# darcamo/pyphysim

Measured on AMD Instinct MI355X. Metric: Monte Carlo realizations/sec (whole node) + SER abs-error vs ref, higher is better.
Workload: dtype f64

## Files before the change

### pyphysim_amd/csrc/capi.hip

```cpp
#include <cmath>
#include <cstdarg>

#include "common.hpp"
#include "modem.hpp"

namespace mcle {

static thread_local char g_err[512] = "";

void set_error(const char* fmt, ...) {
    va_list ap;
    va_start(ap, fmt);
    vsnprintf(g_err, sizeof(g_err), fmt, ap);
    va_end(ap);
}

}

using namespace mcle;

int mcle_ctx::bind() const {
    MCLE_HIP(hipSetDevice(device));
    return MCLE_OK;
}

int mcle_ctx::scratch(size_t bytes, void** d_ptr) {
    if (bytes > scratch_bytes) {
        if (d_scratch) MCLE_HIP(hipFree(d_scratch));
        d_scratch = nullptr;
        scratch_bytes = 0;
        size_t want = bytes < (1u << 20) ? (1u << 20) : (bytes < ((size_t)256 << 20) ? bytes + bytes / 4 : bytes);
        hipError_t e = hipMalloc(&d_scratch, want);
        if (e == hipErrorOutOfMemory && want > bytes) {
            (void)hipGetLastError();
            want = bytes;
            e = hipMalloc(&d_scratch, want);
        }
        if (e != hipSuccess) {
            d_scratch = nullptr;
            MCLE_HIP(e);
        }
        scratch_bytes = want;
    }
    *d_ptr = d_scratch;
    return MCLE_OK;
}

int mcle_ctx::scratch_upto(size_t want, size_t floor_bytes, void** d_ptr, size_t* got) {
    if (want <= scratch_bytes) {
        *d_ptr = d_scratch;
        *got = want;
        return MCLE_OK;
    }
    size_t free_b = 0, total_b = 0;
    if (hipMemGetInfo(&free_b, &total_b) == hipSuccess) {
        const size_t avail = free_b + scratch_bytes;
        const size_t margin = (size_t)256 << 20;
        if (avail > margin && want > avail - margin) want = avail - margin;
    } else {
        (void)hipGetLastError();
    }
    if (want < floor_bytes) want = floor_bytes;
    for (;;) {
        const int rc = scratch(want, d_ptr);
        if (rc == MCLE_OK) {
            *got = want;
            return MCLE_OK;
        }
        if (want <= floor_bytes) return rc;
        (void)hipGetLastError();
        want = want / 2 < floor_bytes ? floor_bytes : want / 2;
    }
}

int mcle_ctx::get_twiddles(int n, int dtype, void** d_tw) {
    TwiddleKey key{n, dtype};
    auto it = twiddles.find(key);
    if (it != twiddles.end()) {
        *d_tw = it->second;
        return MCLE_OK;
    }
    const double two_pi = 6.283185307179586476925286766559;
    void* d = nullptr;
    if (dtype == MCLE_F64) {
        std::vector<double2> h(n);
        for (int k = 0; k < n; ++k) {
            h[k].x = std::cos(two_pi * k / n);
            h[k].y = -std::sin(two_pi * k / n);
        }
        MCLE_HIP(hipMalloc(&d, n * sizeof(double2)));
        MCLE_HIP(hipMemcpy(d, h.data(), n * sizeof(double2), hipMemcpyHostToDevice));
    } else {
        std::vector<float2> h(n);
        for (int k = 0; k < n; ++k) {
            h[k].x = (float)std::cos(two_pi * k / n);
            h[k].y = (float)-std::sin(two_pi * k / n);
        }
        MCLE_HIP(hipMalloc(&d, n * sizeof(float2)));
        MCLE_HIP(hipMemcpy(d, h.data(), n * sizeof(float2), hipMemcpyHostToDevice));
    }
    twiddles[key] = d;
    *d_tw = d;
    return MCLE_OK;
}

extern "C" {

const char* mcle_last_error(void) { return g_err; }

int mcle_version(void) { return MCLE_VERSION; }

int mcle_device_count(int* count) {
    MCLE_REQUIRE(count != nullptr, "null output pointer");
    int n = 0;
    hipError_t e = hipGetDeviceCount(&n);
    if (e != hipSuccess) {
        (void)hipGetLastError();
        n = 0;
    }
    *count = n;
    return MCLE_OK;
}

int mcle_ctx_create(int device_id, mcle_ctx** out) {
    MCLE_REQUIRE(out != nullptr, "null output pointer");
    *out = nullptr;
    int n = 0;
    hipError_t e = hipGetDeviceCount(&n);
    if (e != hipSuccess || n <= 0) {
        (void)hipGetLastError();
        set_error("no HIP device available (hipGetDeviceCount: %s); libmcle has no CPU fallback",
                  e == hipSuccess ? "0 devices" : hipGetErrorString(e));
        return MCLE_E_HIP;
    }
    MCLE_REQUIRE(device_id >= 0 && device_id < n, "device_id %d out of range [0, %d)", device_id, n);
    MCLE_HIP(hipSetDevice(device_id));
    hipDeviceProp_t prop;
    MCLE_HIP(hipGetDeviceProperties(&prop, device_id));
    if (std::strncmp(prop.gcnArchName, "gfx950", 6) != 0) {
        set_error("device %d is %s; libmcle is built for gfx950 (MI355X) only", device_id, prop.gcnArchName);
        return MCLE_E_HIP;
    }
    mcle_ctx* ctx = new (std::nothrow) mcle_ctx();
    if (!ctx) {
        set_error("out of host memory");
        return MCLE_E_NOMEM;
    }
    ctx->device = device_id;
    ctx->n_cu = prop.multiProcessorCount;
    ctx->lds_bytes = (int)prop.sharedMemPerBlock;
    ctx->name = prop.name;
    hipError_t es = hipStreamCreateWithFlags(&ctx->stream, hipStreamNonBlocking);
    if (es != hipSuccess) {
        set_error("hipStreamCreate failed: %s", hipGetErrorString(es));
        delete ctx;
        return MCLE_E_HIP;
    }
    ctx->own_stream = true;
    (void)hipEventCreate(&ctx->ev0);
    (void)hipEventCreate(&ctx->ev1);
    (void)hipEventCreate(&ctx->ev_probe0);
    (void)hipEventCreate(&ctx->ev_probe1);
    *out = ctx;
    return MCLE_OK;
}

int mcle_ctx_destroy(mcle_ctx* ctx) {
    if (!ctx) return MCLE_OK;
    (void)hipSetDevice(ctx->device);
    (void)hipStreamSynchronize(ctx->stream);
    (void)mcle_comm_destroy(ctx);
    if (ctx->d_comm_buf) (void)hipFree(ctx->d_comm_buf);
    for (auto& kv : ctx->twiddles) (void)hipFree(kv.second);
    if (ctx->d_table_f32) (void)hipFree(ctx->d_table_f32);
    if (ctx->d_table_f64) (void)hipFree(ctx->d_table_f64);
    if (ctx->d_grid) (void)hipFree(ctx->d_grid);
    if (ctx->d_psk) (void)hipFree(ctx->d_psk);
    if (ctx->d_scratch) (void)hipFree(ctx->d_scratch);
    if (ctx->ev0) (void)hipEventDestroy(ctx->ev0);
    if (ctx->ev1) (void)hipEventDestroy(ctx->ev1);
    if (ctx->ev_probe0) (void)hipEventDestroy(ctx->ev_probe0);
    if (ctx->ev_probe1) (void)hipEventDestroy(ctx->ev_probe1);
    if (ctx->own_stream && ctx->stream) (void)hipStreamDestroy(ctx->stream);
    delete ctx;
    return MCLE_OK;
}

int mcle_ctx_set_stream(mcle_ctx* ctx, void* hip_stream) {
    MCLE_REQUIRE(ctx != nullptr, "null context");
    MCLE_HIP(hipSetDevice(ctx->device));
    MCLE_HIP(hipStreamSynchronize(ctx->stream));
    if (ctx->own_stream && ctx->stream) MCLE_HIP(hipStreamDestroy(ctx->stream));
    if (hip_stream) {
        ctx->stream = (hipStream_t)hip_stream;
        ctx->own_stream = false;
    } else {
        MCLE_HIP(hipStreamCreateWithFlags(&ctx->stream, hipStreamNonBlocking));
        ctx->own_stream = true;
    }
    return MCLE_OK;
}

int mcle_ctx_get_stream(mcle_ctx* ctx, void** hip_stream) {
    MCLE_REQUIRE(ctx != nullptr && hip_stream != nullptr, "null argument");
    *hip_stream = (void*)ctx->stream;
    return MCLE_OK;
}

int mcle_ctx_set_option(mcle_ctx* ctx, int option, long long value) {
    MCLE_REQUIRE(ctx != nullptr, "null context");
    MCLE_REQUIRE(option >= 0 && option < MCLE_OPT_COUNT, "unknown option %d", option);
    bool ok = false;
    switch (option) {
        case MCLE_OPT_NO_MFMA: case MCLE_OPT_SINGLE_TDL: case MCLE_OPT_JAKES_DIRECT: case MCLE_OPT_F64_GENERIC: case MCLE_OPT_BD_RUNTIME_SOLVE: case MCLE_OPT_DEMOD_NOCERT: case MCLE_OPT_F32_MFMA: case MCLE_OPT_WALK_LEGACY: case MCLE_OPT_STAGED_GENERIC: ok = value == 0 || value == 1; break;
        case MCLE_OPT_TDL_KERNEL: ok = value >= 0 && value <= 4; break;
#ifdef MCLE_EXPERIMENTS
        case MCLE_OPT_MIMO_TDL_KERNEL: ok = value >= 0 && value <= 255; break;
#else
        case MCLE_OPT_MIMO_TDL_KERNEL: ok = value >= 0 && value <= 2; break;
#endif
#ifdef MCLE_EXPERIMENTS
        case MCLE_OPT_F64_VARIANT: ok = value >= 0 && value <= 2047; break;
#else
        case MCLE_OPT_F64_VARIANT:
            MCLE_REQUIRE(value == 0, "option MCLE_OPT_F64_VARIANT: the timing-bound variants are compiled with -DMCLE_EXPERIMENTS only");
            ok = true;
            break;
#endif
        case MCLE_OPT_MFMA_VARIANT: ok = value == 0 || value == 36 || value == 32 || value == 30 || value == 21; break;
        case MCLE_OPT_GRID_OVERSUB: ok = value >= 0 && value <= 64; break;
        case MCLE_OPT_FLAT_WGS_PER_CU: ok = value >= 0 && value <= 4096; break;
        case MCLE_OPT_TDL_MFMA_WAVES: ok = value == 0 || value == 2 || value == 3 || value == 32; break;
        case MCLE_OPT_F64_THREADS: ok = value == 0 || (value >= 256 && value <= 265) || value == 512 || value == 1024; break;
    }
    MCLE_REQUIRE(ok, "option %d: value %lld out of range", option, value);
    ctx->opt[option] = value;
    return MCLE_OK;
}

int mcle_ctx_trim_scratch(mcle_ctx* ctx) {
    MCLE_REQUIRE(ctx != nullptr, "null context");
    MCLE_HIP(hipSetDevice(ctx->device));
    MCLE_HIP(hipStreamSynchronize(ctx->stream));
    if (ctx->d_scratch) MCLE_HIP(hipFree(ctx->d_scratch));
    ctx->d_scratch = nullptr;
    ctx->scratch_bytes = 0;
    return MCLE_OK;
}

int mcle_ctx_get_option(mcle_ctx* ctx, int option, long long* value) {
    MCLE_REQUIRE(ctx != nullptr && value != nullptr, "null argument");
    MCLE_REQUIRE(option >= 0 && option < MCLE_OPT_COUNT, "unknown option %d", option);
    *value = ctx->opt[option];
    return MCLE_OK;
}

int mcle_ctx_sync(mcle_ctx* ctx) {
    MCLE_REQUIRE(ctx != nullptr, "null context");
    MCLE_HIP(hipSetDevice(ctx->device));
    MCLE_HIP(hipStreamSynchronize(ctx->stream));
    return MCLE_OK;
}

int mcle_ctx_device_info(mcle_ctx* ctx, int* n_cu, int* lds_bytes, char* name, int name_len) {
    MCLE_REQUIRE(ctx != nullptr, "null context");
    if (n_cu) *n_cu = ctx->n_cu;
    if (lds_bytes) *lds_bytes = ctx->lds_bytes;
    if (name && name_len > 0) {
        std::strncpy(name, ctx->name.c_str(), name_len - 1);
        name[name_len - 1] = 0;
    }
    return MCLE_OK;
}

int mcle_ctx_last_kernel(mcle_ctx* ctx, char* name, int len) {
    MCLE_REQUIRE(ctx != nullptr && name != nullptr && len > 0, "null argument");
    std::strncpy(name, ctx->last_kernel, len - 1);
    name[len - 1] = 0;
    return MCLE_OK;
}

int mcle_malloc(mcle_ctx* ctx, size_t bytes, void** d_ptr) {
    MCLE_REQUIRE(ctx != nullptr && d_ptr != nullptr, "null argument");
    MCLE_HIP(hipSetDevice(ctx->device));
    *d_ptr = nullptr;
    if (bytes == 0) return MCLE_OK;
    hipError_t e = hipMalloc(d_ptr, bytes);
    if (e != hipSuccess) {
        (void)hipGetLastError();
        set_error("hipMalloc(%zu bytes) failed: %s", bytes, hipGetErrorString(e));
        return MCLE_E_NOMEM;
    }
    return MCLE_OK;
}

int mcle_free(mcle_ctx* ctx, void* d_ptr) {
    MCLE_REQUIRE(ctx != nullptr, "null context");
    if (!d_ptr) return MCLE_OK;
    MCLE_HIP(hipSetDevice(ctx->device));
    MCLE_HIP(hipFree(d_ptr));
    return MCLE_OK;
}

int mcle_memset(mcle_ctx* ctx, void* d_ptr, int value, size_t bytes) {
    MCLE_REQUIRE(ctx != nullptr, "null context");
    if (bytes == 0) return MCLE_OK;
    MCLE_HIP(hipSetDevice(ctx->device));
    MCLE_HIP(hipMemsetAsync(d_ptr, value, bytes, ctx->stream));
    return MCLE_OK;
}

int mcle_memcpy_h2d(mcle_ctx* ctx, void* d_dst, const void* src, size_t bytes) {
    MCLE_REQUIRE(ctx != nullptr, "null context");
    if (bytes == 0) return MCLE_OK;
    MCLE_HIP(hipSetDevice(ctx->device));
    MCLE_HIP(hipMemcpyAsync(d_dst, src, bytes, hipMemcpyHostToDevice, ctx->stream));
    MCLE_HIP(hipStreamSynchronize(ctx->stream));
    return MCLE_OK;
}

int mcle_memcpy_d2h(mcle_ctx* ctx, void* dst, const void* d_src, size_t bytes) {
    MCLE_REQUIRE(ctx != nullptr, "null context");
    if (bytes == 0) return MCLE_OK;
    MCLE_HIP(hipSetDevice(ctx->device));
    MCLE_HIP(hipMemcpyAsync(dst, d_src, bytes, hipMemcpyDeviceToHost, ctx->stream));
    MCLE_HIP(hipStreamSynchronize(ctx->stream));
    return MCLE_OK;
}

int mcle_memcpy_2d(mcle_ctx* ctx, void* d_dst, size_t dst_pitch, const void* d_src, size_t src_pitch,
                   size_t row_bytes, size_t rows) {
    MCLE_REQUIRE(ctx != nullptr, "null context");
    MCLE_REQUIRE(row_bytes <= dst_pitch && row_bytes <= src_pitch, "row_bytes exceeds a pitch");
    if (row_bytes == 0 || rows == 0) return MCLE_OK;
    MCLE_HIP(hipSetDevice(ctx->device));
    MCLE_HIP(hipMemcpy2DAsync(d_dst, dst_pitch, d_src, src_pitch, row_bytes, rows, hipMemcpyDeviceToDevice,
                              ctx->stream));
    return MCLE_OK;
}

int mcle_timer_start(mcle_ctx* ctx) {
    MCLE_REQUIRE(ctx != nullptr, "null context");
    MCLE_HIP(hipSetDevice(ctx->device));
    MCLE_HIP(hipEventRecord(ctx->ev0, ctx->stream));
    return MCLE_OK;
}

int mcle_timer_stop_ms(mcle_ctx* ctx, float* ms) {
    MCLE_REQUIRE(ctx != nullptr && ms != nullptr, "null argument");
    MCLE_HIP(hipSetDevice(ctx->device));
    MCLE_HIP(hipEventRecord(ctx->ev1, ctx->stream));
    MCLE_HIP(hipEventSynchronize(ctx->ev1));
    MCLE_HIP(hipEventElapsedTime(ms, ctx->ev0, ctx->ev1));
    return MCLE_OK;
}

int mcle_build_demod_grid(const double* re_im, int M, int* G_out, double* x0_out, double* y0_out, double* h_out,
                          unsigned long long* cells) {
    MCLE_REQUIRE(re_im != nullptr && G_out != nullptr && x0_out != nullptr && y0_out != nullptr && h_out != nullptr &&
                     cells != nullptr, "null argument");
    MCLE_REQUIRE(M >= 2 && M <= 256, "the candidate grid covers 2 <= M <= 256 (byte indices)");
    int G = 8;
    while (G < 32 && G * G < 4 * M) G *= 2;
    double maxabs = 0.0;
    for (int m = 0; m < 2 * M; ++m) maxabs = std::max(maxabs, std::fabs(re_im[m]));
    MCLE_REQUIRE(maxabs > 0.0, "degenerate constellation");
    const double half = 1.2345 * maxabs;
    const double h = 2.0 * half / G, x0 = -half, y0 = -half;
    const double R = 1.5 * (half + maxabs);
    const double margin = 1e-5 * R * R;
    for (int iy = 0; iy < G; ++iy)
        for (int ix = 0; ix < G; ++ix) {
            const double xl = x0 + ix * h, xh = xl + h, yl = y0 + iy * h, yh = yl + h;
            const double cx_ = 0.5 * (xl + xh), cy_ = 0.5 * (yl + yh);
            int best = 0;
            double bd = 1e300;
            for (int m = 0; m < M; ++m) {
                const double dx = cx_ - re_im[2 * m], dy = cy_ - re_im[2 * m + 1];
                const double d = dx * dx + dy * dy;
                if (d < bd) {
                    bd = d;
                    best = m;
                }
            }
            const double sx = re_im[2 * best], sy = re_im[2 * best + 1];
            unsigned long long word = 0;
            int n = 0;
            for (int m = 0; m < M && n <= 7; ++m) {
                bool keep = (m == best);
                if (!keep) {
                    const double px = re_im[2 * m], py = re_im[2 * m + 1];
                    const double bx = 2.0 * (px - sx), by = 2.0 * (py - sy);
                    const double K = (sx * sx + sy * sy) - (px * px + py * py);
                    const bool inf_x = (bx > 0.0 && ix == G - 1) || (bx < 0.0 && ix == 0);
                    const bool inf_y = (by > 0.0 && iy == G - 1) || (by < 0.0 && iy == 0);
                    if (inf_x || inf_y) {
                        keep = true;
                    } else {
                        const double sup = K + bx * (bx > 0.0 ? xh : xl) + by * (by > 0.0 ? yh : yl);
                        keep = sup >= -margin;
                    }
                }
                if (keep) {
                    if (n < 7) word |= (unsigned long long)m << (8 * (n + 1));
                    ++n;
                }
            }
            cells[iy * G + ix] = n > 7 ? 0xFFull : (word | (unsigned long long)n);
        }
    *G_out = G;
    *x0_out = x0;
    *y0_out = y0;
    *h_out = h;
    return MCLE_OK;
}

int mcle_set_constellation(mcle_ctx* ctx, const double* re_im, int M, int kind) {
    MCLE_REQUIRE(ctx != nullptr && re_im != nullptr, "null argument");
    MCLE_REQUIRE(M >= 2 && M <= 1024 && (M & (M - 1)) == 0, "M must be a power of two in [2, 1024] (got %d)", M);
    MCLE_REQUIRE(kind == MCLE_CONST_GENERIC || kind == MCLE_CONST_QAM || kind == MCLE_CONST_BPSK,
                 "unknown constellation kind %d", kind);
    int bits = 0;
    while ((1 << bits) < M) ++bits;
    double scale = 0.0;
    int L = 0;
    if (kind == MCLE_CONST_QAM) {
        MCLE_REQUIRE(bits % 2 == 0, "M must be a square power of 2");
        L = 1 << (bits / 2);
        scale = std::sqrt((M - 1) * 2.0 / 3.0);
        for (int r = 0; r < L; ++r)
            for (int c = 0; c < L; ++c) {
                const int label = (r << (bits / 2)) | c;
                const int gi = r ^ (r >> 1), gj = c ^ (c >> 1);
                const double re = (-(L - 1) + 2 * gj) / scale, im = ((L - 1) - 2 * gi) / scale;
                MCLE_REQUIRE(std::fabs(re_im[2 * label] - re) < 1e-12 && std::fabs(re_im[2 * label + 1] - im) < 1e-12,
                             "table is not the reference's square Gray %d-QAM (label %d)", M, label);
            }
    }
    MCLE_HIP(hipSetDevice(ctx->device));
    MCLE_HIP(hipStreamSynchronize(ctx->stream));
    if (ctx->d_table_f32) MCLE_HIP(hipFree(ctx->d_table_f32));
    if (ctx->d_table_f64) MCLE_HIP(hipFree(ctx->d_table_f64));
    ctx->d_table_f32 = nullptr;
    ctx->d_table_f64 = nullptr;
    ctx->M = 0;
    std::vector<float2> h32(M);
    for (int m = 0; m < M; ++m) {
        h32[m].x = (float)re_im[2 * m];
        h32[m].y = (float)re_im[2 * m + 1];
    }
    MCLE_HIP(hipMalloc((void**)&ctx->d_table_f32, M * sizeof(float2)));
    MCLE_HIP(hipMalloc((void**)&ctx->d_table_f64, M * sizeof(double2)));
    MCLE_HIP(hipMemcpy(ctx->d_table_f32, h32.data(), M * sizeof(float2), hipMemcpyHostToDevice));
    MCLE_HIP(hipMemcpy(ctx->d_table_f64, re_im, M * sizeof(double2), hipMemcpyHostToDevice));
    ctx->grid_G = 0;
    if (M <= 256) {
        std::vector<unsigned long long> cells(32 * 32);
        int G = 0;
        double x0 = 0, y0 = 0, h = 0;
        int rc = mcle_build_demod_grid(re_im, M, &G, &x0, &y0, &h, cells.data());
        if (rc) return rc;
        if (!ctx->d_grid) MCLE_HIP(hipMalloc((void**)&ctx->d_grid, 32 * 32 * sizeof(unsigned long long)));
        MCLE_HIP(hipMemcpy(ctx->d_grid, cells.data(), (size_t)G * G * sizeof(unsigned long long), hipMemcpyHostToDevice));
        ctx->grid_G = G;
        ctx->grid_x0 = (float)x0;
        ctx->grid_y0 = (float)y0;
        ctx->grid_inv_h = (float)(1.0 / h);
    }
    ctx->M = M;
    ctx->bits = bits;
    ctx->kind = kind;
    ctx->qam_scale = scale;
    ctx->qam_L = L;
    ctx->quad_ok = 0;
    if (M == 4) {
        const double a = std::fabs(re_im[0]), b = std::fabs(re_im[1]);
        unsigned lut = 0, seen = 0;
        bool ok = a > 0.0 && b > 0.0;
        for (int m = 0; m < 4 && ok; ++m) {
            const double re = re_im[2 * m], im = re_im[2 * m + 1];
            ok = std::fabs(std::fabs(re) - a) <= 1e-12 * a && std::fabs(std::fabs(im) - b) <= 1e-12 * b;
            const unsigned q = (re < 0.0 ? 1u : 0u) | (im < 0.0 ? 2u : 0u);
            seen |= 1u << q;
            lut |= (unsigned)m << (8 * q);
        }
        if (ok && seen == 0xFu) {
            ctx->quad_ok = 1;
            ctx->quad_lut = lut;
            ctx->quad_min = a < b ? a : b;
            ctx->quad_max = a < b ? b : a;
        }
    }
    ctx->axis_ok = 0;
    if (M == 4 && !ctx->quad_ok) {
        double a = 0.0;
        for (int i = 0; i < 8; ++i) a = std::fabs(re_im[i]) > a ? std::fabs(re_im[i]) : a;
        unsigned lut = 0, seen = 0;
        bool ok = a > 0.0;
        for (int m = 0; m < 4 && ok; ++m) {
            const double re = re_im[2 * m], im = re_im[2 * m + 1];
            const double big = std::fabs(re) > std::fabs(im) ? std::fabs(re) : std::fabs(im);
            const double small = std::fabs(re) > std::fabs(im) ? std::fabs(im) : std::fabs(re);
            ok = std::fabs(big - a) <= 1e-12 * a && small <= 1e-12 * a;
            const unsigned q = (re - im < 0.0 ? 1u : 0u) | (re + im < 0.0 ? 2u : 0u);
            seen |= 1u << q;
            lut |= (unsigned)m << (8 * q);
        }
        if (ok && seen == 0xFu) {
            ctx->axis_ok = 1;
            ctx->axis_lut = lut;
            ctx->axis_a = a;
        }
    }
    ctx->psk_ok = 0;
    if ((M == 8 || M == 16) && kind != MCLE_CONST_QAM) {
        const double two_pi = 6.283185307179586476925286766559;
        const double rad = std::hypot(re_im[0], re_im[1]);
        bool ok = rad > 0.0;
        double phi0 = 0.0;
        {
            const double a0 = std::atan2(re_im[1], re_im[0]);
            phi0 = std::fmod(a0, two_pi / M);
            if (phi0 < 0.0) phi0 += two_pi / M;
            if (two_pi / M - phi0 < 1e-9) phi0 = 0.0;
        }
// ... 44 lines not shown
```

### pyphysim_amd/csrc/pipeline_mimo_pw.hip

```cpp
#include "mimo_planar_common.hpp"
#include "walk_f64.hpp"

namespace mcle {

constexpr int kPwPlane = 4 * 272;
__host__ __device__ __forceinline__ int pw_slot(int a, int e) { return a * 272 + e + (e >> 4); }
__host__ __device__ __forceinline__ int pw_mtime(int h, int c) { return (c & 3) * 64 + (c >> 2) * 16 + (h & 3) * 4 + (h >> 2); }
template <int NW> constexpr int pw_lab_stride() { return 16 * NW + 16; }

template <int NW, int J, bool STUB>
__device__ __forceinline__ void pw_first_stage(const unsigned char* lab_row, const double2* s_txtab, const double2* __restrict__ g_tw,
                                               double2 (&v)[16]) {
    const uint4* lab = reinterpret_cast<const uint4*>(lab_row);
    if constexpr (NW == 4) {
#pragma unroll
        for (int i = 0; i < 4; ++i) {
            const uint4 L = lab[i];
            const uint32_t wds[4] = {L.x, L.y, L.z, L.w};
#pragma unroll
            for (int uu = 0; uu < 4; ++uu) {
                const int u = 4 * i + uu;
                const uint32_t w = wds[uu];
                double2 X0, X1, X2, X3;
                if constexpr (STUB) {
                    X0 = X1 = X2 = X3 = mk<double>((double)w, 1.0);
                } else {
                    X0 = s_txtab[w & 0xFFu];
                    X1 = s_txtab[(w >> 8) & 0xFFu];
                    X2 = s_txtab[(w >> 16) & 0xFFu];
                    X3 = s_txtab[w >> 24];
                }
                const double2 A = (J & 1) ? csub(X0, X2) : cadd(X0, X2);
                const double2 B = (J & 1) ? csub(X1, X3) : cadd(X1, X3);
                double2 S;
                if constexpr (J == 0) S = cadd(A, B);
                else if constexpr (J == 1) S = mk<double>(A.x - B.y, A.y + B.x);
                else if constexpr (J == 2) S = csub(A, B);
                else S = mk<double>(A.x + B.y, A.y - B.x);
                if constexpr (J == 0) v[u] = S;
                else if (u == 0) v[u] = S;
                else v[u] = cmulc(S, g_tw[16 * J * u]);
            }
        }
    } else if constexpr (NW == 8) {
        constexpr double kH = 0.70710678118654752440;
        auto rotJ = [](double2 z) {
            if constexpr ((J & 3) == 0) return z;
            else if constexpr ((J & 3) == 1) return mk<double>(-z.y, z.x);
            else if constexpr ((J & 3) == 2) return mk<double>(-z.x, -z.y);
            else return mk<double>(z.y, -z.x);
        };
#pragma unroll
        for (int i = 0; i < 8; ++i) {
            const uint4 L = lab[i];
            const uint32_t wds[4] = {L.x, L.y, L.z, L.w};
#pragma unroll
            for (int uu = 0; uu < 2; ++uu) {
                const int u = 2 * i + uu;
                const uint32_t w0 = wds[2 * uu], w1 = wds[2 * uu + 1];
                double2 X[8];
                if constexpr (STUB) {
#pragma unroll
                    for (int q = 0; q < 8; ++q) X[q] = mk<double>((double)(w0 + w1), 1.0);
                } else {
#pragma unroll
                    for (int q = 0; q < 4; ++q) {
                        X[q] = s_txtab[(w0 >> (8 * q)) & 0xFFu];
                        X[q + 4] = s_txtab[(w1 >> (8 * q)) & 0xFFu];
                    }
                }
                double2 A[4];
#pragma unroll
                for (int q = 0; q < 4; ++q) A[q] = (J & 1) ? csub(X[q], X[q + 4]) : cadd(X[q], X[q + 4]);
                const double2 B0 = cadd(A[0], rotJ(A[2])), B1 = cadd(A[1], rotJ(A[3]));
                double2 S;
                if constexpr (J == 0) S = cadd(B0, B1);
                else if constexpr (J == 2) S = mk<double>(B0.x - B1.y, B0.y + B1.x);
                else if constexpr (J == 4) S = csub(B0, B1);
                else if constexpr (J == 6) S = mk<double>(B0.x + B1.y, B0.y - B1.x);
                else {
                    constexpr double c = (J == 1 || J == 7) ? kH : -kH, sn = (J == 1 || J == 3) ? kH : -kH;
                    S = mk<double>(B0.x + (c * B1.x - sn * B1.y), B0.y + (sn * B1.x + c * B1.y));
                }
                if constexpr (J == 0) v[u] = S;
                else if (u == 0) v[u] = S;
                else v[u] = cmulc(S, g_tw[16 * J * u]);
            }
        }
    } else {
        static_assert(NW == 2, "first stage");
#pragma unroll
        for (int i = 0; i < 2; ++i) {
            const uint4 L = lab[i];
            const uint32_t wds[4] = {L.x, L.y, L.z, L.w};
#pragma unroll
            for (int uu = 0; uu < 8; ++uu) {
                const int u = 8 * i + uu;
                const uint32_t w = wds[uu >> 1] >> (16 * (uu & 1));
                double2 X0, X1;
                if constexpr (STUB) {
                    X0 = X1 = mk<double>((double)(w & 0xFFFFu), 1.0);
                } else {
                    X0 = s_txtab[w & 0xFFu];
                    X1 = s_txtab[(w >> 8) & 0xFFu];
                }
                const double2 S = J ? csub(X0, X1) : cadd(X0, X1);
                if constexpr (J == 0) v[u] = S;
                else if (u == 0) v[u] = S;
                else v[u] = cmulc(S, g_tw[16 * J * u]);
            }
        }
    }
}

template <int NW, int DEC, int WPS, bool TD = false, int ABL = 0>
__global__ __launch_bounds__(64 * NW, WPS) void k_run_mimo_ofdm_pw(MimoParams pp, ModemParams<double> mp, uint64_t seed, uint64_t first,
                                                                   uint64_t count, const double2* __restrict__ g_tw,
                                                                   const double2* __restrict__ g_recs, mcle_counters* counters,
                                                                   uint32_t* __restrict__ sym_out, uint32_t* __restrict__ bit_out) {
    using T = double;
    constexpr int N = 256 * NW, NT = 4, NR = 4, kRec = d64_rec<NT, NR>(), TB = 64 * NW, UU = 16 / NW;
    constexpr int kLabStride = pw_lab_stride<NW>();
    static_assert(NW == 2 || NW == 4 || NW == 8, "wavefronts per realization");
    extern __shared__ __attribute__((aligned(16))) char pw_smem[];
    T* s_R = reinterpret_cast<T*>(pw_smem);
    cx<T>* s_table = reinterpret_cast<cx<T>*>(s_R + NW * kPwPlane);
    cx<T>* s_txtab = s_table + ((mp.M + 1) & ~1);
    cx<T>* s_rec = s_txtab + ((mp.M + 1) & ~1);
    unsigned* s_part = reinterpret_cast<unsigned*>(s_rec + 2 * (kRec + 1));
    constexpr int kBm = (kBmLdsDoubles + 1) & ~1;
    double* s_bm = reinterpret_cast<double*>(s_part + 64);
    unsigned char* s_lab = reinterpret_cast<unsigned char*>(s_bm + kBm);

    const int tid = threadIdx.x, lane = tid & 63;
    const int j = __builtin_amdgcn_readfirstlane(tid >> 6);
    const int pj = j & 1;
    const int cp = pp.cp;
    const int per_sym = N * NT;
    const uint64_t row = (uint64_t)pp.n_ofdm_sym * (N + cp);
    const T sigma = (T)sqrt(pp.noise_var);
    const T tx_scale = (T)(1.0 / sqrt((double)NT) / sqrt((double)(N + cp)));
    const T tab_scale = TD ? tx_scale : tx_scale * (T)N;
    const uint32_t mask = (uint32_t)(mp.M - 1);
    for (int m = tid; m < mp.M; m += TB) {
        const cx<T> c = mp.g_table[m];
        s_table[m] = c;
        s_txtab[m] = cscale(c, tab_scale);
    }
    bm_tables_to_lds(s_bm, tid, TB);
    __shared__ WgTotals totals;
    if (tid == 0) wg_zero(totals);

    T* s_mine = s_R + j * kPwPlane;
    uint2* s_words_mine = reinterpret_cast<uint2*>(s_mine);
    uint2* s_words_peer = reinterpret_cast<uint2*>(s_R + (j ^ 1) * kPwPlane);
    uint64_t it = 0, rl_prev = 0;
    cx<T> rec_next = mk<T>(0, 0);
    if (tid < kRec && blockIdx.x < count) rec_next = g_recs[(uint64_t)blockIdx.x * kRec + tid];
    __syncthreads();
    for (uint64_t rl = blockIdx.x; rl < count; rl += gridDim.x, ++it) {
        const Rng rng(seed, first + rl);
        const int buf = (int)(it & 1);
        if (tid < kRec) {
            s_rec[buf * (kRec + 1) + tid] = rec_next;
            if (rl + gridDim.x < count) rec_next = g_recs[(rl + gridDim.x) * kRec + tid];
        }
        const cx<T>* s_H = s_rec + buf * (kRec + 1);
        const cx<T>* s_G = s_H + NT * NR;
        unsigned se = 0, be = 0;
        for (int os = 0; os < pp.n_ofdm_sym; ++os) {
            if (it > 0 || os > 0) __syncthreads();
            {
                const int t = opaque(tid);
                Words4 dw;
                if constexpr (ABL & 32) dw.w[0] = dw.w[1] = dw.w[2] = dw.w[3] = (uint32_t)t * 0x01010101u;
                else dw = rng.block(STREAM_DATA, (uint32_t)(((uint64_t)os * per_sym) >> 4) + (uint32_t)t);
                const int q = (t >> 6) ^ (NW / 2), u = (t & 63) >> 2;
#pragma unroll
                for (int s = 0; s < 4; ++s) {
                    const uint32_t w = dw.w[s] & (mask * 0x01010101u);
                    const int g = 4 * (t & 3) + s;
                    unsigned char* dst = s_lab + g * kLabStride + NW * u + q;
#pragma unroll
                    for (int a = 0; a < 4; ++a) dst[a * 16 * kLabStride] = (unsigned char)(w >> (8 * a));
                }
            }
            {
                const int ln = opaque(lane);
                const int r = ln >> 4, h = ln & 15;
                const uint64_t i00 = (uint64_t)r * row + (uint64_t)os * (N + cp) + cp + (j & ~1) + 32 * NW * pj + NW * (uint64_t)pw_mtime(h, 0);
                const uint32_t b0 = (uint32_t)(i00 >> 1);
                uint2* wm = s_words_mine + (8 * pj) * 64 + ln;
                uint2* wp = s_words_peer + (8 * pj) * 64 + ln;
#pragma unroll
                for (int cc = 0; cc < 8; ++cc) {
                    Words4 b;
                    if constexpr (ABL & 128) b.w[0] = b.w[1] = b.w[2] = b.w[3] = b0 + cc;
                    else b = rng.block(STREAM_NOISE, b0 + (uint32_t)(NW / 2) * (uint32_t)pw_mtime(0, cc));
                    const uint2 even = make_uint2(b.w[0], b.w[1]), odd = make_uint2(b.w[2], b.w[3]);
                    wm[cc * 64] = pj ? odd : even;
                    wp[cc * 64] = pj ? even : odd;
                }
            }
            __syncthreads();
            if (tid == 0 && os == 0 && it > 0) {
                const unsigned* qq = s_part + (buf ^ 1) * 32;
                unsigned ts = 0, tb = 0;
#pragma unroll
                for (int i = 0; i < NW; ++i) {
                    ts += qq[2 * i];
                    tb += qq[2 * i + 1];
                }
                wg_account(totals, ts, tb, s_rec[(buf ^ 1) * (kRec + 1) + 2 * NT * NR].x != 0.0, rl_prev, sym_out, bit_out);
            }
            cx<T> v[16];
            if constexpr (TD) {
                const int ln = opaque(lane);
                const unsigned char* lab = s_lab + ln * kLabStride;
                if constexpr (NW == 4) {
                    switch (j) {
                        case 0: pw_first_stage<4, 0, (ABL & 32) != 0>(lab, s_txtab, g_tw, v); break;
                        case 1: pw_first_stage<4, 1, (ABL & 32) != 0>(lab, s_txtab, g_tw, v); break;
                        case 2: pw_first_stage<4, 2, (ABL & 32) != 0>(lab, s_txtab, g_tw, v); break;
                        default: pw_first_stage<4, 3, (ABL & 32) != 0>(lab, s_txtab, g_tw, v); break;
                    }
                } else if constexpr (NW == 8) {
                    switch (j) {
                        case 0: pw_first_stage<8, 0, (ABL & 32) != 0>(lab, s_txtab, g_tw, v); break;
                        case 1: pw_first_stage<8, 1, (ABL & 32) != 0>(lab, s_txtab, g_tw, v); break;
                        case 2: pw_first_stage<8, 2, (ABL & 32) != 0>(lab, s_txtab, g_tw, v); break;
                        case 3: pw_first_stage<8, 3, (ABL & 32) != 0>(lab, s_txtab, g_tw, v); break;
                        case 4: pw_first_stage<8, 4, (ABL & 32) != 0>(lab, s_txtab, g_tw, v); break;
                        case 5: pw_first_stage<8, 5, (ABL & 32) != 0>(lab, s_txtab, g_tw, v); break;
                        case 6: pw_first_stage<8, 6, (ABL & 32) != 0>(lab, s_txtab, g_tw, v); break;
                        default: pw_first_stage<8, 7, (ABL & 32) != 0>(lab, s_txtab, g_tw, v); break;
                    }
                } else {
                    if (j == 0) pw_first_stage<2, 0, (ABL & 32) != 0>(lab, s_txtab, g_tw, v);
                    else pw_first_stage<2, 1, (ABL & 32) != 0>(lab, s_txtab, g_tw, v);
                }
            }
            if constexpr (TD && !(ABL & 64)) {
                const int g = opaque(lane) & 15;
                R16Tw64<T> tw;
#pragma unroll
                for (int m = 1; m <= 3; ++m) {
                    tw.a1[m - 1] = g_tw[g * (NW * m + j)];
                    tw.a2[m - 1] = g_tw[4 * NW * g * m];
                }
                const cx<T> f0 = g_tw[g * j];
                r16_pass<T, true, false, 0, false, true, true>(nullptr, nullptr, 0, tw, nullptr, 0, v, v);
#pragma unroll
                for (int q = 0; q < 4; ++q) v[q] = cmulc(v[q], f0);
            }
            uint2 nw[16];
            {
                const int ln = opaque(lane);
#pragma unroll
                for (int c = 0; c < 16; ++c) nw[c] = s_words_mine[c * 64 + ln];
            }
            if constexpr (TD) {
                const int ln = opaque(lane);
                const int a = ln >> 4, g = ln & 15;
                const int wbase = pw_slot(a, g), rbase = pw_slot(a, 16 * g);
                T xr[16];
#pragma unroll
                for (int u = 0; u < 16; ++u) s_mine[wbase + 17 * u] = v[u].x;
                walk_wave_order();
#pragma unroll
                for (int c = 0; c < 16; ++c) xr[c] = s_mine[rbase + c];
                walk_wave_order();
#pragma unroll
                for (int u = 0; u < 16; ++u) s_mine[wbase + 17 * u] = v[u].y;
                walk_wave_order();
#pragma unroll
                for (int c = 0; c < 16; ++c) v[c] = mk<T>(xr[c], s_mine[rbase + c]);
            }
            if constexpr (TD && !(ABL & 64)) {
                R16Tw64<T> none;
                r16_pass<T, true, false, 0, false, true, true, false, true>(nullptr, nullptr, 0, none, nullptr, 0, v, v);
            }
            if constexpr (!TD) {
#pragma unroll
                for (int c = 0; c < 16; ++c) {
                    if constexpr (ABL & 128) v[c] = mk<T>((T)nw[c].x, sigma);
                    else v[c] = cn_words(nw[c].x, nw[c].y, sigma, s_bm);
                }
            }
            if constexpr (TD) {
                const int ln = opaque(lane);
                const cx<T> hA = s_H[(ln & 3) * NT + (ln >> 4)];
                const T hre = hA.x, him = hA.y, nhim = -hA.y;
#pragma unroll
                for (int c = 0; c < 16; ++c) {
                    cx<T> z;
                    if constexpr (ABL & 128) z = mk<T>((T)nw[c].x, sigma);
                    else z = cn_words(nw[c].x, nw[c].y, sigma, s_bm);
                    if constexpr (ABL & 256) {
                        v[c] = cadd(v[c], z);
                    } else {
                        T yr = __builtin_amdgcn_mfma_f64_4x4x4f64(hre, v[c].x, z.x, 0, 0, 0);
                        T yi = __builtin_amdgcn_mfma_f64_4x4x4f64(him, v[c].x, z.y, 0, 0, 0);
                        yr = __builtin_amdgcn_mfma_f64_4x4x4f64(nhim, v[c].y, yr, 0, 0, 0);
                        yi = __builtin_amdgcn_mfma_f64_4x4x4f64(hre, v[c].y, yi, 0, 0, 0);
                        v[c] = mk<T>(yr, yi);
                    }
                }
            }
            if constexpr (!(ABL & 512)) {
                R16Tw64<T> none;
                r16_pass<T, false, true, 0, false, true, true, false, true>(nullptr, nullptr, 0, none, nullptr, 0, v, v);
            }
            {
                const int ln = opaque(lane);
                const int a = ln >> 4, g = ln & 15;
                const int wbase = pw_slot(a, g), rbase = pw_slot(a, 16 * g);
                T xr[16];
#pragma unroll
                for (int c = 0; c < 16; ++c) s_mine[rbase + c] = v[c].x;
                walk_wave_order();
#pragma unroll
                for (int u = 0; u < 16; ++u) xr[u] = s_mine[wbase + 17 * u];
                walk_wave_order();
#pragma unroll
                for (int c = 0; c < 16; ++c) s_mine[rbase + c] = v[c].y;
                walk_wave_order();
#pragma unroll
                for (int u = 0; u < 16; ++u) v[u] = mk<T>(xr[u], s_mine[wbase + 17 * u]);
            }
            if constexpr (!(ABL & 512)) {
                const int g = opaque(lane) & 15;
                R16Tw64<T> tw;
#pragma unroll
                for (int m = 1; m <= 3; ++m) {
                    tw.a1[m - 1] = g_tw[NW * g * m];
                    tw.a2[m - 1] = g_tw[4 * NW * g * m];
                }
                r16_pass<T, false, true, 0, false, true, true>(nullptr, nullptr, 0, tw, nullptr, 0, v, v);
            }
            T er[NW][UU], ei[NW][UU];
            {
                const int ln = opaque(lane);
                const int r = ln >> 4, g = ln & 15;
                const int wpos = r * 272 + g, rpos = r * 272 + g + 16 * UU * j;
                r16_wave_sync();
#pragma unroll
                for (int u = 0; u < 16; ++u) s_mine[wpos + 16 * u] = v[u].x;
                __syncthreads();
#pragma unroll
                for (int jj = 0; jj < NW; ++jj)
#pragma unroll
                    for (int uu = 0; uu < UU; ++uu) er[jj][uu] = s_R[jj * kPwPlane + rpos + 16 * uu];
                __syncthreads();
#pragma unroll
                for (int u = 0; u < 16; ++u) s_mine[wpos + 16 * u] = v[u].y;
                __syncthreads();
#pragma unroll
                for (int jj = 0; jj < NW; ++jj)
#pragma unroll
                    for (int uu = 0; uu < UU; ++uu) ei[jj][uu] = s_R[jj * kPwPlane + rpos + 16 * uu];
            }
            if constexpr (!(ABL & 1024)) {
                const int ln = opaque(lane);
                const int g = ln & 15;
#pragma unroll
                for (int uu = 0; uu < UU; ++uu) {
                    const int kp = g + 16 * (UU * j + uu);
                    if constexpr (NW == 4) {
                        const cx<T> w1 = g_tw[kp], w2 = g_tw[2 * kp], w3 = g_tw[3 * kp];
                        const cx<T> u0 = mk<T>(er[0][uu], ei[0][uu]);
                        const cx<T> u1 = cmul(mk<T>(er[1][uu], ei[1][uu]), w1);
                        const cx<T> u2 = cmul(mk<T>(er[2][uu], ei[2][uu]), w2);
                        const cx<T> u3 = cmul(mk<T>(er[3][uu], ei[3][uu]), w3);
                        CxOps<T>::template bfly4<false>(u0, u1, u2, u3, v[4 * uu], v[4 * uu + 1], v[4 * uu + 2], v[4 * uu + 3]);
                    } else if constexpr (NW == 8) {
                        cx<T> x[8];
                        x[0] = mk<T>(er[0][uu], ei[0][uu]);
#pragma unroll
                        for (int jj = 1; jj < 8; ++jj) x[jj] = cmul(mk<T>(er[jj][uu], ei[jj][uu]), g_tw[jj * kp]);
                        cx<T> E[4], O[4];
                        CxOps<T>::template bfly4<false>(x[0], x[2], x[4], x[6], E[0], E[1], E[2], E[3]);
                        CxOps<T>::template bfly4<false>(x[1], x[3], x[5], x[7], O[0], O[1], O[2], O[3]);
                        constexpr T kH = (T)0.70710678118654752440;
                        const cx<T> t0 = O[0];
                        const cx<T> t1 = mk<T>(kH * (O[1].x + O[1].y), kH * (O[1].y - O[1].x));
                        const cx<T> t2 = mk<T>(O[2].y, -O[2].x);
                        const cx<T> t3 = mk<T>(kH * (O[3].y - O[3].x), -kH * (O[3].x + O[3].y));
                        v[8 * uu + 0] = cadd(E[0], t0); v[8 * uu + 4] = csub(E[0], t0);
                        v[8 * uu + 1] = cadd(E[1], t1); v[8 * uu + 5] = csub(E[1], t1);
                        v[8 * uu + 2] = cadd(E[2], t2); v[8 * uu + 6] = csub(E[2], t2);
                        v[8 * uu + 3] = cadd(E[3], t3); v[8 * uu + 7] = csub(E[3], t3);
                    } else {
                        const cx<T> u0 = mk<T>(er[0][uu], ei[0][uu]);
                        const cx<T> u1 = cmul(mk<T>(er[1][uu], ei[1][uu]), g_tw[kp]);
                        v[2 * uu] = cadd(u0, u1);
                        v[2 * uu + 1] = csub(u0, u1);
                    }
                }
            }
            {
                const int ln = opaque(lane);
                const uint4 L = *reinterpret_cast<const uint4*>(s_lab + ln * kLabStride + 16 * j);
                const uint32_t wds[4] = {L.x, L.y, L.z, L.w};
                if constexpr (!TD && !(ABL & 256)) {
                    const cx<T> hA = s_H[(ln & 3) * NT + (ln >> 4)];
                    const T hre = hA.x, him = hA.y, nhim = -hA.y;
#pragma unroll
                    for (int u = 0; u < 16; ++u) {
                        const uint32_t lb = (wds[u >> 2] >> (8 * (u & 3))) & 0xFFu;
                        cx<T> X;
                        if constexpr (ABL & 32) X = mk<T>((T)lb, 1.0);
                        else X = s_txtab[lb];
                        T yr = __builtin_amdgcn_mfma_f64_4x4x4f64(hre, X.x, v[u].x, 0, 0, 0);
                        T yi = __builtin_amdgcn_mfma_f64_4x4x4f64(him, X.x, v[u].y, 0, 0, 0);
                        yr = __builtin_amdgcn_mfma_f64_4x4x4f64(nhim, X.y, yr, 0, 0, 0);
                        yi = __builtin_amdgcn_mfma_f64_4x4x4f64(hre, X.y, yi, 0, 0, 0);
                        v[u] = mk<T>(yr, yi);
                    }
                }
                if constexpr (!(ABL & 1024)) {
                const cx<T> gA = s_G[(ln & 3) * NR + (ln >> 4)];
                const T gre = gA.x, gim = gA.y, ngim = -gA.y;
#pragma unroll
                for (int i = 0; i < 4; ++i) {
                    cx<T> e[4];
                    int tx[4];
#pragma unroll
                    for (int jj = 0; jj < 4; ++jj) {
                        const int u = 4 * i + jj;
                        T xr = __builtin_amdgcn_mfma_f64_4x4x4f64(gre, v[u].x, 0.0, 0, 0, 0);
                        T xi = __builtin_amdgcn_mfma_f64_4x4x4f64(gim, v[u].x, 0.0, 0, 0, 0);
                        xr = __builtin_amdgcn_mfma_f64_4x4x4f64(ngim, v[u].y, xr, 0, 0, 0);
                        xi = __builtin_amdgcn_mfma_f64_4x4x4f64(gre, v[u].y, xi, 0, 0, 0);
                        e[jj] = mk<T>(xr, xi);
                        tx[jj] = (int)((wds[i] >> (8 * jj)) & 0xFFu);
                    }
                    walk_decide<DEC, 4>(mp, s_table, nullptr, e, tx, se, be);
                }
                } else {
                    T keep = er[0][0] + ei[NW - 1][UU - 1];
                    if constexpr (!TD) {
#pragma unroll
                        for (int u = 0; u < 16; ++u) keep += v[u].x + v[u].y;
                    }
                    se += (unsigned)(keep == 0.5) + (wds[0] == 0x12345u);
                }
            }
        }
        se = wave_sum_u32(se);
        be = wave_sum_u32(be);
        if (lane == 0) {
            s_part[buf * 32 + 2 * j] = se;
            s_part[buf * 32 + 2 * j + 1] = be;
        }
        rl_prev = rl;
    }
    __syncthreads();
    if (tid == 0) {
        if (it > 0) {
            const int buf = (int)((it - 1) & 1);
            const unsigned* qq = s_part + buf * 32;
            unsigned ts = 0, tb = 0;
#pragma unroll
            for (int i = 0; i < NW; ++i) {
                ts += qq[2 * i];
                tb += qq[2 * i + 1];
            }
            wg_account(totals, ts, tb, s_rec[buf * (kRec + 1) + 2 * NT * NR].x != 0.0, rl_prev, sym_out, bit_out);
        }
        wg_flush(totals, counters, (unsigned long long)per_sym * pp.n_ofdm_sym, (unsigned long long)per_sym * pp.n_ofdm_sym * mp.bits);
    }
}

template <int NW, int WPS, bool TD = false, int ABL = 0>
static int launch_mimo_ofdm_pw(mcle_ctx* ctx, const mcle_mimo_ofdm_cfg* cfg, uint64_t seed, uint64_t first, uint64_t count,
                               mcle_counters* d_counters, uint32_t* d_sym, uint32_t* d_bit) {
    using T = double;
    constexpr int N = 256 * NW, NT = 4, NR = 4, kRec = d64_rec<NT, NR>();
    int rc;
    void* tw = nullptr;
    if ((rc = ctx->get_twiddles(N, MCLE_F64, &tw))) return rc;
    MimoParams pp{cfg->cp_size, cfg->num_used, cfg->n_ofdm_sym, cfg->mmse, cfg->noise_var};
    ModemParams<T> mp = pipe_modem<T>(ctx, cfg->demod_method);
    const int dec = walk_dec_kind(ctx, mp);
    mp.grid.G = 0;
    const size_t tab_len = ((size_t)mp.M + 1) & ~(size_t)1;
    const size_t lds = (size_t)NW * kPwPlane * sizeof(T) + (2 * tab_len + 2 * (kRec + 1)) * sizeof(cx<T>) + 64 * sizeof(unsigned) +
                       (size_t)((kBmLdsDoubles + 1) & ~1) * sizeof(double) + (size_t)64 * pw_lab_stride<NW>();
    MCLE_REQUIRE(lds + 512 <= (size_t)160 * 1024, "part-wave MIMO-OFDM kernel: %zu B of LDS do not fit", lds);
    auto kern = k_run_mimo_ofdm_pw<NW, WDEC_SLICER, WPS, TD, ABL>;
    switch (dec) {
        case WDEC_QAM_CERT: kern = k_run_mimo_ofdm_pw<NW, WDEC_QAM_CERT, WPS, TD, ABL>; break;
        case WDEC_QUAD_CERT: kern = k_run_mimo_ofdm_pw<NW, WDEC_QUAD_CERT, WPS, TD, ABL>; break;
        case WDEC_AXIS4_CERT: kern = k_run_mimo_ofdm_pw<NW, WDEC_AXIS4_CERT, WPS, TD, ABL>; break;
        default: break;
    }
    MCLE_HIP(hipFuncSetAttribute((const void*)kern, hipFuncAttributeMaxDynamicSharedMemorySize, (int)lds));
    int per_cu = (int)((size_t)160 * 1024 / (lds + 512));
    if (per_cu < 1) per_cu = 1;
    const int by_waves = WPS * 4 / NW;
    if (per_cu > by_waves) per_cu = by_waves;
    const uint64_t resident = (uint64_t)ctx->n_cu * per_cu;
    ctx->set_kernel("mimo_ofdm_pw<%d>/%s%s", NW, TD ? "time" : "freq", WPS == (NW == 8 ? 2 : 3) ? "" : "/w2");
    const uint64_t kSlice = 1ull << 20;
    const uint64_t slice = count < kSlice ? count : kSlice;
    void* recs = nullptr;
    if ((rc = ctx->scratch((size_t)slice * kRec * sizeof(cx<T>), &recs))) return rc;
    for (uint64_t off = 0; off < count; off += slice) {
        const uint64_t n = count - off < slice ? count - off : slice;
        hipLaunchKernelGGL((k_mimo_filters_planar<T, N, NT, NR>), dim3((unsigned)((n + 63) / 64)), dim3(64), 0, ctx->stream, pp, seed,
                           first + off, n, (cx<T>*)recs);
        MCLE_LAUNCH_CHECK();
        const unsigned grid = (unsigned)oversubscribed_grid(ctx, resident, n, 8, NW == 4 ? 32 : 16);
        hipLaunchKernelGGL(kern, dim3(grid), dim3(64 * NW), lds, ctx->stream, pp, mp, seed, first + off, n, (const cx<T>*)tw,
                           (const cx<T>*)recs, d_counters, d_sym ? d_sym + off : nullptr, d_bit ? d_bit + off : nullptr);
        MCLE_LAUNCH_CHECK();
    }
    return MCLE_OK;
}

int run_mimo_ofdm_pw(mcle_ctx* ctx, const mcle_mimo_ofdm_cfg* cfg, uint64_t seed, uint64_t first, uint64_t count,
                     mcle_counters* d_counters, uint32_t* d_sym, uint32_t* d_bit) {
    if (!((cfg->fft_size == 512 || cfg->fft_size == 1024 || cfg->fft_size == 2048) && cfg->nt == 4 && cfg->nr == 4 && cfg->num_used == cfg->fft_size &&
          (cfg->cp_size & 1) == 0))
        return MCLE_E_UNSUPPORTED;
    if (ctx->M > 256) return MCLE_E_UNSUPPORTED;
    {
        ModemParams<double> mp = pipe_modem<double>(ctx, cfg->demod_method);
        if (walk_dec_kind(ctx, mp) == WDEC_GENERIC) return MCLE_E_UNSUPPORTED;
    }
    const bool two = ctx->opt[MCLE_OPT_F64_THREADS] == 262 || ctx->opt[MCLE_OPT_F64_THREADS] == 264;
    const bool td = ctx->opt[MCLE_OPT_F64_THREADS] == 265;
    if (cfg->fft_size == 2048) {
        return td ? launch_mimo_ofdm_pw<8, 2, true>(ctx, cfg, seed, first, count, d_counters, d_sym, d_bit)
                  : launch_mimo_ofdm_pw<8, 2>(ctx, cfg, seed, first, count, d_counters, d_sym, d_bit);
    }
#ifdef MCLE_EXPERIMENTS
#define MCLE_PW_ABL(NW_, V_)                                                                                          \
    case V_:                                                                                                          \
        return td ? launch_mimo_ofdm_pw<NW_, 3, true, V_>(ctx, cfg, seed, first, count, d_counters, d_sym, d_bit)     \
                  : launch_mimo_ofdm_pw<NW_, 3, false, V_>(ctx, cfg, seed, first, count, d_counters, d_sym, d_bit);
#define MCLE_PW_ABLS(NW_)                                                                                             \
    switch ((int)ctx->opt[MCLE_OPT_F64_VARIANT]) {                                                                    \
        MCLE_PW_ABL(NW_, 32) MCLE_PW_ABL(NW_, 64) MCLE_PW_ABL(NW_, 128) MCLE_PW_ABL(NW_, 256) MCLE_PW_ABL(NW_, 512)   \
        MCLE_PW_ABL(NW_, 1024) MCLE_PW_ABL(NW_, 2016)                                                                 \
        default: break;                                                                                               \
    }
#else
#define MCLE_PW_ABLS(NW_)
#endif
    if (cfg->fft_size == 512) {
        MCLE_PW_ABLS(2)
        if (td) return launch_mimo_ofdm_pw<2, 3, true>(ctx, cfg, seed, first, count, d_counters, d_sym, d_bit);
        return two ? launch_mimo_ofdm_pw<2, 2>(ctx, cfg, seed, first, count, d_counters, d_sym, d_bit)
                   : launch_mimo_ofdm_pw<2, 3>(ctx, cfg, seed, first, count, d_counters, d_sym, d_bit);
    }
    MCLE_PW_ABLS(4)
#undef MCLE_PW_ABLS
#ifdef MCLE_EXPERIMENTS
#undef MCLE_PW_ABL
#endif
    if (td) return launch_mimo_ofdm_pw<4, 3, true>(ctx, cfg, seed, first, count, d_counters, d_sym, d_bit);
    return two ? launch_mimo_ofdm_pw<4, 2>(ctx, cfg, seed, first, count, d_counters, d_sym, d_bit)
               : launch_mimo_ofdm_pw<4, 3>(ctx, cfg, seed, first, count, d_counters, d_sym, d_bit);
}

}
```

Measured before the change: 41.39 million.

## Keep own-wave data in registers during LDS exchanges in MIMO OFDM kernel

In the frequency-domain path, each wave now keeps its own half of the noise words in registers instead of writing them to LDS and reading them back. In the cross-wave exchange, each wave skips the LDS round-trip for its own slice by dispatching on a compile-time wave index. The realization loop counter is narrowed to 32 bits. New experiment ablation variants (2048, 4064) are also added. This trims LDS traffic and 64-bit index arithmetic, at the cost of extra register pressure and code duplication across the per-wave switch.

```diff
diff --git a/pyphysim_amd/csrc/capi.hip b/pyphysim_amd/csrc/capi.hip
--- a/pyphysim_amd/csrc/capi.hip
+++ b/pyphysim_amd/csrc/capi.hip
@@ -220,7 +220,7 @@
         case MCLE_OPT_MIMO_TDL_KERNEL: ok = value >= 0 && value <= 2; break;
 #endif
 #ifdef MCLE_EXPERIMENTS
-        case MCLE_OPT_F64_VARIANT: ok = value >= 0 && value <= 2047; break;
+        case MCLE_OPT_F64_VARIANT: ok = value >= 0 && value <= 4095; break;
 #else
         case MCLE_OPT_F64_VARIANT:
             MCLE_REQUIRE(value == 0, "option MCLE_OPT_F64_VARIANT: the timing-bound variants are compiled with -DMCLE_EXPERIMENTS only");
diff --git a/pyphysim_amd/csrc/pipeline_mimo_pw.hip b/pyphysim_amd/csrc/pipeline_mimo_pw.hip
--- a/pyphysim_amd/csrc/pipeline_mimo_pw.hip
+++ b/pyphysim_amd/csrc/pipeline_mimo_pw.hip
@@ -3,6 +3,7 @@
 
 namespace mcle {
 
+constexpr uint64_t kPwSlice = 1ull << 20;
 constexpr int kPwPlane = 4 * 272;
 __host__ __device__ __forceinline__ int pw_slot(int a, int e) { return a * 272 + e + (e >> 4); }
 __host__ __device__ __forceinline__ int pw_mtime(int h, int c) { return (c & 3) * 64 + (c >> 2) * 16 + (h & 3) * 4 + (h >> 2); }
@@ -113,6 +114,54 @@
     }
 }
 
+template <int NW, class F>
+__device__ __forceinline__ void pw_by_class(int j, F&& f) {
+    static_assert(NW == 2 || NW == 4 || NW == 8, "wavefronts per realization");
+    if constexpr (NW == 2) {
+        if (j == 0) f(std::integral_constant<int, 0>{});
+        else f(std::integral_constant<int, 1>{});
+    } else if constexpr (NW == 4) {
+        switch (j) {
+            case 0: f(std::integral_constant<int, 0>{}); break;
+            case 1: f(std::integral_constant<int, 1>{}); break;
+            case 2: f(std::integral_constant<int, 2>{}); break;
+            default: f(std::integral_constant<int, 3>{}); break;
+        }
+    } else {
+        switch (j) {
+            case 0: f(std::integral_constant<int, 0>{}); break;
+            case 1: f(std::integral_constant<int, 1>{}); break;
+            case 2: f(std::integral_constant<int, 2>{}); break;
+            case 3: f(std::integral_constant<int, 3>{}); break;
+            case 4: f(std::integral_constant<int, 4>{}); break;
+            case 5: f(std::integral_constant<int, 5>{}); break;
+            case 6: f(std::integral_constant<int, 6>{}); break;
+            default: f(std::integral_constant<int, 7>{}); break;
+        }
+    }
+}
+
+template <int NW, int J, int SEL>
+__device__ __forceinline__ void pw_exchange_write(double* s_mine, int wpos, const double2 (&v)[16]) {
+    constexpr int UU = 16 / NW;
+#pragma unroll
+    for (int u = 0; u < 16; ++u)
+        if (u / UU != J) s_mine[wpos + 16 * u] = SEL ? v[u].y : v[u].x;
+    __builtin_amdgcn_wave_barrier();
+}
+template <int NW, int J, int SEL>
+__device__ __forceinline__ void pw_exchange_read(const double* s_R, int pos, int rpos, const double2 (&v)[16], double (&e)[NW][16 / NW]) {
+    constexpr int UU = 16 / NW;
+#pragma unroll
+    for (int jj = 0; jj < NW; ++jj)
+#pragma unroll
+        for (int uu = 0; uu < UU; ++uu) {
+            if (jj == J) e[jj][uu] = SEL ? v[UU * (J < 0 ? 0 : J) + uu].y : v[UU * (J < 0 ? 0 : J) + uu].x;
+            else e[jj][uu] = s_R[jj * kPwPlane + (J < 0 ? rpos : pos + 16 * UU * J) + 16 * uu];
+        }
+    __builtin_amdgcn_wave_barrier();
+}
+
 template <int NW, int DEC, int WPS, bool TD = false, int ABL = 0>
 __global__ __launch_bounds__(64 * NW, WPS) void k_run_mimo_ofdm_pw(MimoParams pp, ModemParams<double> mp, uint64_t seed, uint64_t first,
                                                                    uint64_t count, const double2* __restrict__ g_tw,
@@ -121,6 +170,7 @@
     using T = double;
     constexpr int N = 256 * NW, NT = 4, NR = 4, kRec = d64_rec<NT, NR>(), TB = 64 * NW, UU = 16 / NW;
     constexpr int kLabStride = pw_lab_stride<NW>();
+    constexpr bool kOwnShare = NW != 8;
     static_assert(NW == 2 || NW == 4 || NW == 8, "wavefronts per realization");
     extern __shared__ __attribute__((aligned(16))) char pw_smem[];
     T* s_R = reinterpret_cast<T*>(pw_smem);
@@ -154,16 +204,17 @@
     T* s_mine = s_R + j * kPwPlane;
     uint2* s_words_mine = reinterpret_cast<uint2*>(s_mine);
     uint2* s_words_peer = reinterpret_cast<uint2*>(s_R + (j ^ 1) * kPwPlane);
-    uint64_t it = 0, rl_prev = 0;
+    const uint32_t cnt = (uint32_t)count;
+    uint32_t it = 0, rl_prev = 0;
     cx<T> rec_next = mk<T>(0, 0);
     if (tid < kRec && blockIdx.x < count) rec_next = g_recs[(uint64_t)blockIdx.x * kRec + tid];
     __syncthreads();
-    for (uint64_t rl = blockIdx.x; rl < count; rl += gridDim.x, ++it) {
+    for (uint32_t rl = blockIdx.x; rl < cnt; rl += gridDim.x, ++it) {
         const Rng rng(seed, first + rl);
         const int buf = (int)(it & 1);
         if (tid < kRec) {
             s_rec[buf * (kRec + 1) + tid] = rec_next;
-            if (rl + gridDim.x < count) rec_next = g_recs[(rl + gridDim.x) * kRec + tid];
+            if (rl + gridDim.x < cnt) rec_next = g_recs[(uint64_t)(rl + gridDim.x) * kRec + tid];
         }
         const cx<T>* s_H = s_rec + buf * (kRec + 1);
         const cx<T>* s_G = s_H + NT * NR;
@@ -185,21 +236,23 @@
                     for (int a = 0; a < 4; ++a) dst[a * 16 * kLabStride] = (unsigned char)(w >> (8 * a));
                 }
             }
+            uint2 nw_own[8];
             {
                 const int ln = opaque(lane);
                 const int r = ln >> 4, h = ln & 15;
                 const uint64_t i00 = (uint64_t)r * row + (uint64_t)os * (N + cp) + cp + (j & ~1) + 32 * NW * pj + NW * (uint64_t)pw_mtime(h, 0);
                 const uint32_t b0 = (uint32_t)(i00 >> 1);
                 uint2* wm = s_words_mine + (8 * pj) * 64 + ln;
-                uint2* wp = s_words_peer + (8 * pj) * 64 + ln;
+                uint2* wp = s_words_peer + (TD ? 8 * pj : 0) * 64 + ln;
 #pragma unroll
                 for (int cc = 0; cc < 8; ++cc) {
                     Words4 b;
                     if constexpr (ABL & 128) b.w[0] = b.w[1] = b.w[2] = b.w[3] = b0 + cc;
                     else b = rng.block(STREAM_NOISE, b0 + (uint32_t)(NW / 2) * (uint32_t)pw_mtime(0, cc));
                     const uint2 even = make_uint2(b.w[0], b.w[1]), odd = make_uint2(b.w[2], b.w[3]);
-                    wm[cc * 64] = pj ? odd : even;
-                    wp[cc * 64] = pj ? even : odd;
+                    if constexpr (TD) wm[cc * 64] = pj ? odd : even;
+                    else nw_own[cc] = pj ? odd : even;
+                    if constexpr (TD || !(ABL & 2048)) wp[cc * 64] = pj ? even : odd;
                 }
             }
             __syncthreads();
@@ -254,10 +307,23 @@
                 for (int q = 0; q < 4; ++q) v[q] = cmulc(v[q], f0);
             }
             uint2 nw[16];
-            {
+            if constexpr (TD) {
                 const int ln = opaque(lane);
 #pragma unroll
                 for (int c = 0; c < 16; ++c) nw[c] = s_words_mine[c * 64 + ln];
+            } else {
+                const int ln = opaque(lane);
+                uint2 got[8];
+#pragma unroll
+                for (int cc = 0; cc < 8; ++cc) {
+                    if constexpr (ABL & 2048) got[cc] = nw_own[cc];
+                    else got[cc] = s_words_mine[cc * 64 + ln];
+                }
+#pragma unroll
+                for (int cc = 0; cc < 8; ++cc) {
+                    nw[cc] = pj ? got[cc] : nw_own[cc];
+                    nw[8 + cc] = pj ? nw_own[cc] : got[cc];
+                }
             }
             if constexpr (TD) {
                 const int ln = opaque(lane);
@@ -314,19 +380,21 @@
             {
                 const int ln = opaque(lane);
                 const int a = ln >> 4, g = ln & 15;
-                const int wbase = pw_slot(a, g), rbase = pw_slot(a, 16 * g);
-                T xr[16];
-#pragma unroll
-                for (int c = 0; c < 16; ++c) s_mine[rbase + c] = v[c].x;
-                walk_wave_order();
-#pragma unroll
-                for (int u = 0; u < 16; ++u) xr[u] = s_mine[wbase + 17 * u];
-                walk_wave_order();
-#pragma unroll
-                for (int c = 0; c < 16; ++c) s_mine[rbase + c] = v[c].y;
-                walk_wave_order();
-#pragma unroll
-                for (int u = 0; u < 16; ++u) v[u] = mk<T>(xr[u], s_mine[wbase + 17 * u]);
+                if constexpr (!(ABL & 2048)) {
+                    const int wbase = pw_slot(a, g), rbase = pw_slot(a, 16 * g);
+                    T xr[16];
+#pragma unroll
+                    for (int c = 0; c < 16; ++c) s_mine[rbase + c] = v[c].x;
+                    walk_wave_order();
+#pragma unroll
+                    for (int u = 0; u < 16; ++u) xr[u] = s_mine[wbase + 17 * u];
+                    walk_wave_order();
+#pragma unroll
+                    for (int c = 0; c < 16; ++c) s_mine[rbase + c] = v[c].y;
+                    walk_wave_order();
+#pragma unroll
+                    for (int u = 0; u < 16; ++u) v[u] = mk<T>(xr[u], s_mine[wbase + 17 * u]);
+                }
             }
             if constexpr (!(ABL & 512)) {
                 const int g = opaque(lane) & 15;
@@ -339,26 +407,40 @@
                 r16_pass<T, false, true, 0, false, true, true>(nullptr, nullptr, 0, tw, nullptr, 0, v, v);
             }
             T er[NW][UU], ei[NW][UU];
-            {
+            if constexpr (ABL & 2048) {
+#pragma unroll
+                for (int jj = 0; jj < NW; ++jj)
+#pragma unroll
+                    for (int uu = 0; uu < UU; ++uu) {
+                        er[jj][uu] = v[UU * jj + uu].x;
+                        ei[jj][uu] = v[UU * jj + uu].y;
+                    }
+                __syncthreads();
+                __syncthreads();
+                __syncthreads();
+            } else {
                 const int ln = opaque(lane);
                 const int r = ln >> 4, g = ln & 15;
-                const int wpos = r * 272 + g, rpos = r * 272 + g + 16 * UU * j;
+                const int pos = r * 272 + g;
+                const int rpos = pos + 16 * UU * j;
                 r16_wave_sync();
-#pragma unroll
-                for (int u = 0; u < 16; ++u) s_mine[wpos + 16 * u] = v[u].x;
-                __syncthreads();
-#pragma unroll
-                for (int jj = 0; jj < NW; ++jj)
-#pragma unroll
-                    for (int uu = 0; uu < UU; ++uu) er[jj][uu] = s_R[jj * kPwPlane + rpos + 16 * uu];
-                __syncthreads();
-#pragma unroll
-                for (int u = 0; u < 16; ++u) s_mine[wpos + 16 * u] = v[u].y;
-                __syncthreads();
-#pragma unroll
-                for (int jj = 0; jj < NW; ++jj)
-#pragma unroll
-                    for (int uu = 0; uu < UU; ++uu) ei[jj][uu] = s_R[jj * kPwPlane + rpos + 16 * uu];
+                if constexpr (kOwnShare) {
+                    pw_by_class<NW>(j, [&](auto J) __attribute__((always_inline)) { pw_exchange_write<NW, decltype(J)::value, 0>(s_mine, pos, v); });
+                    __syncthreads();
+                    pw_by_class<NW>(j, [&](auto J) __attribute__((always_inline)) { pw_exchange_read<NW, decltype(J)::value, 0>(s_R, pos, rpos, v, er); });
+                    __syncthreads();
+                    pw_by_class<NW>(j, [&](auto J) __attribute__((always_inline)) { pw_exchange_write<NW, decltype(J)::value, 1>(s_mine, pos, v); });
+                    __syncthreads();
+                    pw_by_class<NW>(j, [&](auto J) __attribute__((always_inline)) { pw_exchange_read<NW, decltype(J)::value, 1>(s_R, pos, rpos, v, ei); });
+                } else {
+                    pw_exchange_write<NW, -1, 0>(s_mine, pos, v);
+                    __syncthreads();
+                    pw_exchange_read<NW, -1, 0>(s_R, pos, rpos, v, er);
+                    __syncthreads();
+                    pw_exchange_write<NW, -1, 1>(s_mine, pos, v);
+                    __syncthreads();
+                    pw_exchange_read<NW, -1, 1>(s_R, pos, rpos, v, ei);
+                }
             }
             if constexpr (!(ABL & 1024)) {
                 const int ln = opaque(lane);
@@ -502,7 +584,7 @@
     if (per_cu > by_waves) per_cu = by_waves;
     const uint64_t resident = (uint64_t)ctx->n_cu * per_cu;
     ctx->set_kernel("mimo_ofdm_pw<%d>/%s%s", NW, TD ? "time" : "freq", WPS == (NW == 8 ? 2 : 3) ? "" : "/w2");
-    const uint64_t kSlice = 1ull << 20;
+    const uint64_t kSlice = kPwSlice;
     const uint64_t slice = count < kSlice ? count : kSlice;
     void* recs = nullptr;
     if ((rc = ctx->scratch((size_t)slice * kRec * sizeof(cx<T>), &recs))) return rc;
@@ -543,7 +625,7 @@
 #define MCLE_PW_ABLS(NW_)                                                                                             \
     switch ((int)ctx->opt[MCLE_OPT_F64_VARIANT]) {                                                                    \
         MCLE_PW_ABL(NW_, 32) MCLE_PW_ABL(NW_, 64) MCLE_PW_ABL(NW_, 128) MCLE_PW_ABL(NW_, 256) MCLE_PW_ABL(NW_, 512)   \
-        MCLE_PW_ABL(NW_, 1024) MCLE_PW_ABL(NW_, 2016)                                                                 \
+        MCLE_PW_ABL(NW_, 1024) MCLE_PW_ABL(NW_, 2016) MCLE_PW_ABL(NW_, 2048) MCLE_PW_ABL(NW_, 4064)                   \
         default: break;                                                                                               \
     }
 #else
```

Measured after the change: 42.23 million (median of 6 runs). 2.0% higher.
